# danielwillemsen/alphazero-openspiel

Hardware: AMD Instinct MI355X
Metric: self-play games/sec (higher is better)
Workload: dtype f32-grade (f16x3: split-fp16 operands, 3 MFMAs per product, fp32 accumulate); 1 GPU; connect_four, 400 sims/move, 10-block x 50-filter ResNet, 4096 concurrent games per GPU; overlap=1, weights=random-init (torch.manual_seed), eval-mode BN, net_backend=fused, tree_dtype=f64, parallelism=games sharded over 1 GPU(s), no collective inside the search, hip_graph=True, ticks_per_graph=16, workload_key=connect_four|4096|400|10|50|fused|random|f32x|1|16|build:5fb6d05c6dce

## Files before the change

### alphazero-openspiel_amd/csrc/az_head.h

```cpp
#pragma once
#include "az_head_params.h"

__device__ __forceinline__ half8 frag_from_rows(half8 v, int lane) {
    typedef int i32x4 __attribute__((ext_vector_type(4)));
    const int src = (4 * (lane & 15) + (lane >> 4)) * 4;
    i32x4 u = __builtin_bit_cast(i32x4, v);
#pragma unroll
    for (int i = 0; i < 4; i++) u[i] = __builtin_amdgcn_ds_bpermute(src, u[i]);
    return __builtin_bit_cast(half8, u);
}

template <bool X3> __global__ __launch_bounds__(HEAD_NW * 64) void az_head_kernel(HeadParams p) {
    extern __shared__ __attribute__((aligned(16))) unsigned char lds[];
    float *part = (float *)lds;
    float *logits = (float *)(lds + HEAD_NW * OTG * 64 * 16);
    const int tid = threadIdx.x, lane = tid & 63, wave = tid >> 6;
    const int b0 = blockIdx.x * 16;
    const int K = p.K, NP = p.n_ot * 16;
    int row = b0 + (lane >> 2);
    if (row >= p.n_boards) row = p.n_boards - 1;
    const _Float16 *xrow = p.x + (size_t)row * K + 8 * (lane & 3);
    const _Float16 *xrow_lo = X3 ? p.x_lo + (size_t)row * K + 8 * (lane & 3) : nullptr;
    for (int og = 0; og < p.n_ot; og += OTG) {
        f32x4 acc[OTG], acc2[X3 ? OTG : 1];
#pragma unroll
        for (int o = 0; o < OTG; o++) acc[o] = (f32x4){0.f, 0.f, 0.f, 0.f};
#pragma unroll
        for (int o = 0; o < (X3 ? OTG : 1); o++) acc2[o] = (f32x4){0.f, 0.f, 0.f, 0.f};
        if (p.n_ot == 1) {
#pragma unroll 8
            for (int ks = wave; ks < p.ksteps; ks += HEAD_NW) {
                half8 a = frag_from_rows(*(const half8 *)(xrow + 32 * ks), lane);
                half8 w = *(const half8 *)(p.fc_w + ((size_t)ks * 64 + lane) * 8);
                acc[0] = __builtin_amdgcn_mfma_f32_16x16x32_f16(a, w, acc[0], 0, 0, 0);
                if constexpr (X3) {
                    half8 al = frag_from_rows(*(const half8 *)(xrow_lo + 32 * ks), lane);
                    half8 wl = *(const half8 *)(p.fc_w_lo + ((size_t)ks * 64 + lane) * 8);
                    acc2[0] = __builtin_amdgcn_mfma_f32_16x16x32_f16(a, wl, acc2[0], 0, 0, 0);
                    acc2[0] = __builtin_amdgcn_mfma_f32_16x16x32_f16(al, w, acc2[0], 0, 0, 0);
                }
            }
        } else
        for (int ks = wave; ks < p.ksteps; ks += HEAD_NW) {
            half8 a = frag_from_rows(*(const half8 *)(xrow + 32 * ks), lane);
            half8 al;
            if constexpr (X3) al = frag_from_rows(*(const half8 *)(xrow_lo + 32 * ks), lane);
#pragma unroll
            for (int o = 0; o < OTG; o++)
                if (og + o < p.n_ot) {
                    const size_t wi = (((size_t)(og + o) * p.ksteps + ks) * 64 + lane) * 8;
                    half8 w = *(const half8 *)(p.fc_w + wi);
                    acc[o] = __builtin_amdgcn_mfma_f32_16x16x32_f16(a, w, acc[o], 0, 0, 0);
                    if constexpr (X3) {
                        half8 wl = *(const half8 *)(p.fc_w_lo + wi);
                        acc2[o] = __builtin_amdgcn_mfma_f32_16x16x32_f16(a, wl, acc2[o], 0, 0, 0);
                        acc2[o] = __builtin_amdgcn_mfma_f32_16x16x32_f16(al, w, acc2[o], 0, 0, 0);
                    }
                }
        }
#pragma unroll
        for (int o = 0; o < OTG; o++) {
            if constexpr (X3) acc[o] = acc[o] + acc2[o] * (1.0f / 2048.0f);
            *(f32x4 *)(part + ((wave * OTG + o) * 64 + lane) * 4) = acc[o];
        }
        __syncthreads();
        for (int s = tid; s < OTG * 64; s += HEAD_NW * 64) {
            int o = s >> 6, ln = s & 63;
            if (og + o >= p.n_ot) continue;
            f32x4 v = *(f32x4 *)(part + ((0 * OTG + o) * 64 + ln) * 4);
#pragma unroll
            for (int w = 1; w < HEAD_NW; w++) v += *(f32x4 *)(part + ((w * OTG + o) * 64 + ln) * 4);
            int col = 16 * (og + o) + (ln & 15);
            float bias = p.fc_b[col];
#pragma unroll
            for (int r = 0; r < 4; r++) logits[((ln >> 4) * 4 + r) * NP + col] = v[r] + bias;
        }
        __syncthreads();
    }
    const int brd = (tid >> 4) & 15, sub = tid & 15;
    const float *lg = logits + brd * NP;
    float mx = -INFINITY;
    for (int o = sub; o < p.A; o += 16) mx = fmaxf(mx, lg[o]);
#pragma unroll
    for (int off = 8; off; off >>= 1) mx = fmaxf(mx, __shfl_xor(mx, off, 16));
    float sum = 0.f;
    for (int o = sub; o < p.A; o += 16) sum += X3 ? expf(lg[o] - mx) : __expf(lg[o] - mx);
#pragma unroll
    for (int off = 8; off; off >>= 1) sum += __shfl_xor(sum, off, 16);
    if (tid < 256 && b0 + brd < p.n_boards) {
        float *out = p.priors + (size_t)(b0 + brd) * p.A;
        if (X3) {
            for (int o = sub; o < p.A; o += 16) out[o] = expf(lg[o] - mx) / sum;
        } else {
            float inv = 1.f / sum;
            for (int o = sub; o < p.A; o += 16) out[o] = __expf(lg[o] - mx) * inv;
        }
        if (sub == 0) p.values[b0 + brd] = tanhf(lg[p.A]);
    }
}

#define HG_BT 8
#define HG_OT 8
#define HG_KSPLIT 2
#define HG_RING 4
#ifndef HG_LOADERS
#define HG_LOADERS 4
#endif
template <bool X3> __global__ __launch_bounds__((8 + HG_LOADERS) * 64) void az_head_gemm_kernel(HeadParams p, float *__restrict__ logits_g) {
    extern __shared__ __attribute__((aligned(16))) unsigned char lds[];
    constexpr int NPART = X3 ? 2 : 1;
    constexpr int PIECES = (HG_BT + HG_OT) * NPART;
    constexpr int SLOT_B = PIECES * 1024;
    constexpr int NLOAD = HG_LOADERS;
    constexpr int PER = PIECES / NLOAD;
    static_assert((NLOAD == 2 || NLOAD == 4) && PIECES % NLOAD == 0 && HG_BT == 8 && HG_OT == 8 && (HG_RING - 2) * PER < 64, "piece f = NLOAD i + loader; the counted waits fit vmcnt");
    const int tid = threadIdx.x, lane = tid & 63, wave = __builtin_amdgcn_readfirstlane(tid >> 6), q = lane >> 4, l15 = lane & 15;
    const int wm = (wave & 7) >> 1, wn = (wave ^ (wave >> 2)) & 1;
    const int n_cg = (p.n_ot + HG_OT - 1) / HG_OT, ot_per = (p.n_ot + n_cg - 1) / n_cg, per_bt = n_cg * HG_KSPLIT;
    const int lin = blockIdx.x, xcd = lin & 7, j = lin >> 3;
    const int bt = (j / per_bt) * 8 + xcd;
    if (bt * 16 * HG_BT >= p.n_boards) return;
    const int og = ((j % per_bt) / HG_KSPLIT) * ot_per, kh = (j % per_bt) % HG_KSPLIT;
    const int n_og = p.n_ot - og < ot_per ? p.n_ot - og : ot_per;
    const int K = p.K, NP = p.n_ot * 16;
    const int ks_per = (p.ksteps + HG_KSPLIT - 1) / HG_KSPLIT, ks0 = kh * ks_per;
    const int nk = (p.ksteps - ks0 < ks_per ? p.ksteps - ks0 : ks_per);
    const bool loader = wave >= 8;
    const _Float16 *src0[PER];
    int kstride[PER], dst[PER];
    if (loader) {
#pragma unroll
        for (int i = 0; i < PER; i++) {
            const int f = NLOAD * i + (wave & (NLOAD - 1));
            dst[i] = f * 1024;
            if (f < HG_BT * NPART) {
                const int r = lane >> 2;
                int row = (bt * HG_BT + f % HG_BT) * 16 + r;
                if (row >= p.n_boards) row = p.n_boards - 1;
                src0[i] = (f / HG_BT ? p.x_lo : p.x) + (size_t)row * K + 8 * ((lane & 3) ^ ((r >> 3) << 1));
                kstride[i] = 32;
            } else {
                const int g = f - HG_BT * NPART;
                int ot = og + g % HG_OT;
                ot = ot < p.n_ot ? ot : p.n_ot - 1;
                src0[i] = (g / HG_OT ? p.fc_w_lo : p.fc_w) + ((size_t)ot * p.ksteps * 64 + lane) * 8;
                kstride[i] = 512;
            }
        }
    }
    auto issue = [&](int ks, int slot) {
#pragma unroll
        for (int i = 0; i < PER; i++)
            __builtin_amdgcn_global_load_lds((const __attribute__((address_space(1))) void *)(src0[i] + (size_t)ks * kstride[i]),
                                             (__attribute__((address_space(3))) void *)(lds + slot * SLOT_B + dst[i]), 16, 0, 0);
    };
    if (loader) {
#pragma unroll
        for (int s = 0; s < HG_RING - 1; s++)
            if (s < nk) issue(ks0 + s, s);
        for (int i = -1; i < nk; i++) {
            if (i + 1 < nk) {
                const int younger = nk - 2 - i < HG_RING - 2 ? nk - 2 - i : HG_RING - 2;
                static_for<HG_RING - 1>([&](auto y_c) {
                    constexpr int y = decltype(y_c)::value;
                    if (younger == y) asm volatile("s_waitcnt vmcnt(%0)" ::"n"(y * PER) : "memory");
                });
            }
            __builtin_amdgcn_s_barrier();
            asm volatile("" ::: "memory");
            if (i + HG_RING < nk) issue(ks0 + i + HG_RING, (i + HG_RING) % HG_RING);
        }
        return;
    }
    const int n_m = (bt * HG_BT + 2 * wm + 1) * 16 < p.n_boards ? 2 : (bt * HG_BT + 2 * wm) * 16 < p.n_boards ? 1 : 0;
    const int n_o = n_og - 4 * wn < 0 ? 0 : n_og - 4 * wn > 4 ? 4 : n_og - 4 * wn;
    float bias_o[4];
#pragma unroll
    for (int o = 0; o < 4; o++) bias_o[o] = kh == 0 && o < n_o ? p.fc_b[16 * (og + 4 * wn + o) + l15] : 0.f;
    f32x4 acc[2][4], acc2[X3 ? 2 : 1][X3 ? 4 : 1];
#pragma unroll
    for (int m = 0; m < 2; m++)
#pragma unroll
        for (int o = 0; o < 4; o++) {
            acc[m][o] = (f32x4){0.f, 0.f, 0.f, 0.f};
            if constexpr (X3) acc2[m][o] = (f32x4){0.f, 0.f, 0.f, 0.f};
        }
    const int a_off = (4 * l15 + (q ^ ((l15 >> 3) << 1))) * 16 + 2 * wm * 1024;
    const int w_off = (HG_BT * NPART + 4 * wn) * 1024 + lane * 16;
    auto kloop = [&](auto no_c) {
        constexpr int NO = decltype(no_c)::value, NOT = NO ? NO : 4;
        half8 af[2], afl[X3 ? 2 : 1], w[4], wl[X3 ? 4 : 1];
        auto read = [&](int i) {
            const unsigned char *sb = lds + (i % HG_RING) * SLOT_B;
#pragma unroll
            for (int m = 0; m < 2; m++) {
                af[m] = *(const half8 *)(sb + a_off + m * 1024);
                if constexpr (X3) afl[m] = *(const half8 *)(sb + a_off + (HG_BT + m) * 1024);
            }
#pragma unroll
            for (int o = 0; o < NOT; o++) {
                w[o] = *(const half8 *)(sb + w_off + o * 1024);
                if constexpr (X3) wl[o] = *(const half8 *)(sb + w_off + (HG_OT + o) * 1024);
            }
        };
        auto step = [&](int i) {
            read(i);
#pragma unroll
            for (int pass = 0; pass < (X3 ? 3 : 1); pass++)
#pragma unroll
                for (int o = 0; o < NOT; o++)
#pragma unroll
                    for (int m = 0; m < 2; m++)
// ... 76 lines not shown
```

### alphazero-openspiel_amd/csrc/az_head_params.h

```cpp
#pragma once
#include "az_net_common.h"

struct HeadParams {
    int HW, A, n_ot, ksteps, n_boards;
    int K;
    const _Float16 *x;
    const _Float16 *fc_w;
    const _Float16 *x_lo, *fc_w_lo;
    const float *fc_b;
    float *priors, *values;
};

#define OTG 8
#define HEAD_NW 8

hipError_t az_launch_tower_f16(int device, int nt, int ck, int waves, int r3, const TowerParams &tp, int grid, int lds, hipStream_t st);
hipError_t az_launch_tower_f16c(int device, int ck, const TowerParams &tp, int n_boards, int lds, hipStream_t st);
hipError_t az_launch_tower_x3(int device, int nt, bool rp1, int r3, const TowerParams &tp, int grid, int lds, hipStream_t st);
hipError_t az_launch_tower_x3b(int device, const TowerParams &tp, int grid, hipStream_t st);
hipError_t az_launch_tower_x3d(int device, int variant, const TowerParams &tp, int grid, hipStream_t st);
struct X3DVariant { int pc, tiles, rs, R; };
constexpr int AZ_X3D_VARIANTS = 3;
constexpr X3DVariant az_x3d_variant(int v) { return v == 0 ? X3DVariant{480, 18, 8, 58} : v == 1 ? X3DVariant{416, 16, 9, 84} : X3DVariant{480, 21, 8, 57}; }
hipError_t az_launch_tower_x3c(int device, int bpw, const TowerParams &tp, int n_boards, hipStream_t st);
hipError_t az_launch_head(int device, bool x3, const HeadParams &hp, int n_boards, int lds_head, float *logits, hipStream_t st);
```

### alphazero-openspiel_amd/csrc/az_net.hip

```cpp
#include <hip/hip_runtime.h>
#include <stdint.h>
#include <string.h>

#include <algorithm>
#include <cmath>

#include <string>
#include <vector>

#include "../../include/az_engine.h"
#include "../../include/az_net.h"

#include "az_net_common.h"
#include "az_head_params.h"
#include "az_net_wide.h"

#define AZ_X3C_MAX_BOARDS 512
#define AZ_F16C_MAX_BOARDS 512
#define AZ_X3C_ONE_PER_WG 256

enum class NetScheme {
    F16,
    F16C,
    X3,
// ... 284 lines not shown
    if (out.variant < 0) return out;
    const X3DVariant V = az_x3d_variant(out.variant);
    const int ncol = 16 * V.tiles;
    out.pos.assign(ncol, 0);
    std::vector<int> col_of((size_t)out.nb * HW, -1), seen(16, 0);
    for (int b = 0; b < out.nb; b++)
        for (int pp = 0; pp < HW; pp++) {
            const int r = (b * out.R + (pp / W + 1) * out.rs + pp % W + 1) & 15, k = seen[r]++;
            out.pos[k * 16 + r] = (uint16_t)(b << 8 | pp);
            col_of[(size_t)b * HW + pp] = k * 16 + r;
        }
    out.sdst.assign((size_t)ncol * 8, 0xFFFF);
    for (int col = 0; col < ncol; col++) {
        const int b = out.pos[col] >> 8, pp = out.pos[col] & 255, y = pp / W, x = pp % W;
        for (int t = 0; t < 8; t++) {
            const int tap = X3D::tap_of_plane(t), dy = tap / 3 - 1, dx = tap % 3 - 1, yd = y - dy, xd = x - dx;
            if (yd >= 0 && yd < H && xd >= 0 && xd < W) out.sdst[(size_t)col * 8 + t] = (uint16_t)col_of[(size_t)b * HW + yd * W + xd];
        }
    }
    return out;
}

static std::vector<uint16_t> repack_fc(const uint16_t *src, int n_ot, int fc_ksteps, int HW, int xc) {
    const int ks64 = HW * AZ_NET_XOUT_C / 32;
    std::vector<uint16_t> dst((size_t)n_ot * fc_ksteps * 64 * 8, 0);
    for (int ot = 0; ot < n_ot; ot++)
        for (int ks = 0; ks < fc_ksteps; ks++)
            for (int lane = 0; lane < 64; lane++)
                for (int e = 0; e < 8; e++) {
                    const int k = 32 * ks + 8 * (lane >> 4) + e;
                    if (k >= HW * xc) continue;
                    const int k64 = (k / xc) * AZ_NET_XOUT_C + k % xc;
                    dst[(((size_t)ot * fc_ksteps + ks) * 64 + lane) * 8 + e] =
                        src[(((size_t)ot * ks64 + k64 / 32) * 64 + ((k64 % 32) / 8) * 16 + (lane & 15)) * 8 + k64 % 8];
                }
    return dst;
}

template <bool IS_FIRST> static constexpr int x3b_mfma_per_tile() {
    int n = 0;
    for (int ks = 0; ks < X3BK<IS_FIRST, 1>::NKSC; ks++) n += X3BK<IS_FIRST, 1>::n_mfma(ks);
    return n;
}
static_assert(x3b_mfma_per_tile<false>() == 147, "az_tower_x3b.h: 147 against 180");
static double x3_mfma_per_wave(int nt, int n_convs, int nks) { return 3.0 * (AZ_NET_K0STEPS + (double)(n_convs - 1) * nks) * 4 * nt; }

static std::string head_label(const az_net *n) {
    const std::string t = n->precision == AZ_NET_PREC_F16X3 ? "<X3>" : "";
    return n->n_ot > OTG ? "az_head_gemm_kernel" + t + " + az_head_softmax_kernel" + t : "az_head_kernel" + t;
}
static std::string kind_label(const az_net *n, TowerKind k) {
    std::string s = TOWER_NAME[(int)k];
    if (k == TowerKind::WIDE) s += std::string(n->precision == AZ_NET_PREC_F16X3 ? "<X3>" : "<F16>") + " x" + std::to_string(2 * n->d.n_blocks);
    return k == TowerKind::X3C_FUSED_HEAD ? s : s + " + " + head_label(n);
}

template <class Desc> static int check_args(const Desc *desc, az_net **out, const char *desc_name) {
    if (!desc || !out) {
        g_net_err = "null argument";
        return AZ_E_INVALID;
    }
    *out = nullptr;
    if (desc->struct_size != (int32_t)sizeof(Desc)) {
        g_net_err = std::string(desc_name) + ".struct_size mismatch";
        return AZ_E_INVALID;
    }
    return AZ_OK;
}
static int new_net(int device, az_net **n) {
    const hipError_t s = hipSetDevice(device);
    if (s != hipSuccess) {
        g_net_err = std::string("hipSetDevice: ") + hipGetErrorString(s);
        return AZ_E_HIP;
    }
    *n = new az_net();
    return AZ_OK;
}
struct Upload {
    int rc = AZ_OK;
    void fail(int code, const char *msg) {
        if (rc != AZ_OK) return;
        g_net_err = msg;
        rc = code;
    }
    template <class T> void operator()(T *&dst, const void *src, size_t bytes) {
        if (rc == AZ_OK && (hipMalloc((void **)&dst, bytes) != hipSuccess || hipMemcpy(dst, src, bytes, hipMemcpyHostToDevice) != hipSuccess))
            fail(AZ_E_NOMEM, "hipMalloc/hipMemcpy of the net's weights failed");
    }
};
static int finish_create(az_net *n, const Upload &up, az_net **out) {
    if (up.rc != AZ_OK) {
        az_net_destroy(n);
        return up.rc;
    }
    for (int k = 0; k < N_TOWER_KINDS; k++) n->labels[k] = kind_label(n, (TowerKind)k);
    *out = n;
    return AZ_OK;
}

extern "C" int az_net_create(const az_net_desc *desc, az_net **out) {
    if (int rc = check_args(desc, out, "az_net_desc")) return rc;
    const az_net_desc &d = *desc;
    if (d.rows < 3 || d.cols < 3 || d.rows * d.cols > 64 || d.in_planes < 1 || d.in_planes > 4 || d.n_filters < 1 ||
        d.n_filters > AZ_NET_CPAD || d.n_blocks < 1 || d.num_actions < 1 || !d.conv_w || !d.conv_epi || !d.in_affine ||
        !d.skip_w || !d.fc_w || !d.fc_b) {
        g_net_err = "bad net description (need 3<=rows,cols, rows*cols<=64, in_planes<=4, n_filters<=56, packed buffers)";
        return AZ_E_INVALID;
    }
    if (d.precision != AZ_NET_PREC_F16 && d.precision != AZ_NET_PREC_F16X3) {
        g_net_err = "precision must be AZ_NET_PREC_F16 or AZ_NET_PREC_F16X3";
        return AZ_E_INVALID;
    }
    const bool x3 = d.precision == AZ_NET_PREC_F16X3;
    if (x3 && (!d.conv_w_lo || !d.fc_w_lo)) {
        g_net_err = "AZ_NET_PREC_F16X3 needs conv_w_lo and fc_w_lo";
        return AZ_E_INVALID;
    }
    const int r3 = d.n_filters <= 50 ? 2 : 16, HW = d.rows * d.cols;
    NetScheme scheme;
    X3DLayout xd;
    if (x3) {
        const TowerGeom g = x3_geom(d.rows, d.cols, r3);
        const bool x3b = g.rp1 && r3 == 2;
        if (!x3b && (g.nt > 4 || g.lds > 160 * 1024)) {
            g_net_err = "board / filter count does not fit the f16x3 tower kernel's LDS budget";
            return AZ_E_INVALID;
        }
        if (r3 == 2) xd = x3d_layout(d.rows, d.cols);
        scheme = xd.variant >= 0 ? (x3b ? NetScheme::X3B_X3D : NetScheme::X3D) : x3b ? NetScheme::X3B : NetScheme::X3;
    } else {
        const TowerGeom gc = tower_geom(1, 1, d.rows, d.cols);
        scheme = r3 == 2 && gc.tpb && gc.rs == 8 && gc.tpb <= 3 ? NetScheme::F16C : NetScheme::F16;
    }
    int best = 0;
    for (int bpw = 1; bpw <= 8; bpw++) {
        TowerGeom g = tower_geom(bpw, 4, d.rows, d.cols);
        if (g.nt > 4 || g.lds > 160 * 1024) break;
        best = bpw;
    }
    if (!best) {
        g_net_err = "board does not fit the tower kernel's LDS budget";
        return AZ_E_INVALID;
    }
    az_net *n;
    if (int rc = new_net(d.device, &n)) return rc;
    n->d = d;
    n->precision = d.precision;
    n->scheme = scheme;
    n->r3 = r3;
    memcpy(n->in_affine, d.in_affine, sizeof n->in_affine);
    n->bpw_max = best;
    n->n_ot = (d.num_actions + 1 + 15) / 16;
    n->lds_head = HEAD_NW * OTG * 64 * 16 + 16 * n->n_ot * 16 * 4;
    n->xc = (n->n_ot > OTG && HW % 2 == 0 && d.n_filters <= 52) ? 52 : AZ_NET_XOUT_C;
    n->fc_ksteps = (HW * n->xc + 31) / 32;
    Upload up;
    const int n_convs = 2 * d.n_blocks;
    auto x3_stream = [&](const X3Stream &L, _Float16 *&dst) {
        std::vector<unsigned char> s;
        if (!build_x3_stream(L, d.conv_w, d.conv_w_lo, n_convs, s))
            up.fail(AZ_E_INVALID, "AZ_NET_PREC_F16X3: a conv weight of magnitude >= 32 (the device copy holds the weights x 2048 in fp16)");
        up(dst, s.data(), s.size());
    };
    if (xd.variant >= 0) {
        n->xd_variant = xd.variant, n->xd_nb = xd.nb, n->xd_R = xd.R, n->xd_rs = xd.rs;
        x3_stream(x3d_stream_layout(), n->conv_w_d);
        up(n->xd_pos, xd.pos.data(), xd.pos.size() * 2);
        up(n->xd_sdst, xd.sdst.data(), xd.sdst.size() * 2);
    }
    if (scheme == NetScheme::X3B || scheme == NetScheme::X3B_X3D) x3_stream(x3b_stream_layout(), n->conv_w);
    else {
        const std::vector<unsigned char> s = conv_stream(d, r3);
        up(n->conv_w, s.data(), s.size());
    }
    {
        std::vector<float> e4((size_t)n_convs * 256, 0.f);
        for (int c = 0; c < n_convs; c++) {
            memcpy(&e4[(size_t)c * 256], d.conv_epi + (size_t)c * 192, 192 * sizeof(float));
            if (c + 1 < n_convs) memcpy(&e4[(size_t)c * 256 + 192], d.conv_epi + (size_t)(c + 1) * 192, 64 * sizeof(float));
            if (x3)
                for (int i = 0; i < 64; i++) e4[(size_t)c * 256 + 192 + i] *= X3_WSCALE;
        }
        up(n->epi, e4.data(), e4.size() * sizeof(float));
    }
    const size_t fw = (size_t)n->n_ot * n->fc_ksteps * 64 * 8 * 2;
    for (int lo = 0; lo < (x3 ? 2 : 1); lo++) {
        const uint16_t *src = lo ? d.fc_w_lo : d.fc_w;
        std::vector<uint16_t> re;
        if (n->xc != AZ_NET_XOUT_C) re = repack_fc(src, n->n_ot, n->fc_ksteps, HW, n->xc), src = re.data();
        up(lo ? n->fc_w_lo : n->fc_w, src, fw);
    }
    up(n->fc_b, d.fc_b, (size_t)n->n_ot * 16 * 4);
    up(n->skip_w, d.skip_w, 64 * 4 * sizeof(float));
    n->d.conv_w_lo = nullptr;
    n->d.fc_w_lo = nullptr;
    n->d.conv_w = nullptr;
    n->d.conv_epi = nullptr;
    n->d.in_affine = nullptr;
    n->d.skip_w = nullptr;
    n->d.fc_w = nullptr;
    n->d.fc_b = nullptr;
    return finish_create(n, up, out);
}

static int wide_fpad(int f) { return (f + 31) & ~31; }
static int wide_nks(const az_net *n, int conv) { return conv == 0 ? 9 : 9 * n->fpad / 32; }

extern "C" int az_net_create_wide(const az_net_wide_desc *desc, az_net **out) {
    if (int rc = check_args(desc, out, "az_net_wide_desc")) return rc;
    const az_net_wide_desc &d = *desc;
    if (d.rows < 1 || d.cols < 1 || d.rows * d.cols > 64 || d.in_planes < 1 || d.in_planes > 4 || d.n_filters < 1 ||
        d.n_filters > AZ_NET_WIDE_MAX_FILTERS || d.n_blocks < 1 || d.num_actions < 1 || d.num_actions > 768 || !d.conv_w ||
        !d.conv_b || !d.bn1_scale || !d.bn1_shift || !d.skip_w || !d.fc_w || !d.fc_b) {
        g_net_err = "bad wide net description (need rows*cols<=64, 1<=in_planes<=4, 1<=n_filters<=256, A<=768, all buffers)";
        return AZ_E_INVALID;
    }
    if (d.precision != AZ_NET_PREC_F16 && d.precision != AZ_NET_PREC_F16X3) {
        g_net_err = "precision must be AZ_NET_PREC_F16 or AZ_NET_PREC_F16X3";
        return AZ_E_INVALID;
    }
    const int F = d.n_filters, HW = d.rows * d.cols, cin0 = d.in_planes, C = F > cin0 ? F : cin0, nc = 2 * d.n_blocks;
    const int fpad = wide_fpad(F), nmt = fpad / 16, A1 = d.num_actions + 1;
    const size_t n_w = (size_t)nc * F * C * 9;
    for (size_t i = 0; i < n_w; i++)
        if (!std::isfinite(d.conv_w[i])) {
            g_net_err = "az_net_create_wide: a conv weight is not finite";
            return AZ_E_INVALID;
        }
    az_net *n;
    if (int rc = new_net(d.device, &n)) return rc;
    n->d = az_net_desc{};
    n->d.struct_size = sizeof(az_net_desc);
    n->d.rows = d.rows, n->d.cols = d.cols, n->d.in_planes = cin0, n->d.n_filters = F, n->d.n_blocks = d.n_blocks;
    n->d.num_actions = d.num_actions, n->d.device = d.device, n->d.precision = d.precision;
    n->precision = d.precision;
    n->scheme = NetScheme::WIDE;
    n->fpad = fpad;
    n->nbw = 16 * WIDE_NT / HW;
    n->xc = fpad;
    n->n_ot = (A1 + 15) / 16;
    n->fc_ksteps = HW * fpad / 32;
    n->lds_head = HEAD_NW * OTG * 64 * 16 + 16 * n->n_ot * 16 * 4;
    std::vector<uint16_t> w;
    std::vector<float> epi((size_t)nc * 4 * fpad, 0.f);
    auto h16 = [](double v) {
        _Float16 h = (_Float16)v;
        uint16_t b;
        memcpy(&b, &h, 2);
        return b;
    };
    for (int c = 0; c < nc; c++) {
        n->w_off.push_back(w.size());
        const int cin = c == 0 ? WIDE_CIN0 : fpad, n_ch = cin / 32, cin_real = c == 0 ? cin0 : F;
        const float *wc = d.conv_w + (size_t)c * F * C * 9;
        std::vector<double> sc(fpad, 1.0);
        for (int co = 0; co < F; co++) {
            double m = 0;
            for (int k = 0; k < cin_real * 9; k++) m = std::max(m, (double)std::fabs(wc[((size_t)co * C + k / 9) * 9 + k % 9]));
            int e = 0;
            if (m > 0) {
                (void)std::frexp(m, &e);
                e = std::min(100, std::max(-100, 4 - e));
            }
            sc[co] = std::ldexp(1.0, e);
        }
        const size_t base = w.size();
        w.resize(base + (size_t)n_ch * 9 * nmt * 2 * 512, 0);
        for (int ch = 0; ch < n_ch; ch++)
            for (int tap = 0; tap < 9; tap++)
                for (int mt = 0; mt < nmt; mt++)
                    for (int lane = 0; lane < 64; lane++)
                        for (int j = 0; j < 8; j++) {
                            const int co = 16 * mt + (lane & 15), ci = 32 * ch + 8 * (lane >> 4) + j;
                            if (co >= F || ci >= cin_real) continue;
                            const double v = (double)wc[((size_t)co * C + ci) * 9 + tap] * sc[co];
                            const double hi = (double)(_Float16)v;
                            const size_t o = base + ((((size_t)(ch * 9 + tap) * nmt + mt) * 2) * 512) + lane * 8 + j;
                            w[o] = h16(hi * 2048.0);
                            w[o + 512] = h16((v - hi) * 2048.0);
                        }
        float *e4 = &epi[(size_t)c * 4 * fpad];
        for (int co = 0; co < fpad; co++) e4[co] = (float)(1.0 / (2048.0 * sc[co]));
        for (int co = 0; co < F; co++) {
            e4[fpad + co] = d.conv_b[(size_t)c * F + co];
            if (c % 2 == 1 && c + 1 < nc) {
                e4[2 * fpad + co] = d.bn1_scale[(size_t)(c / 2 + 1) * C + co];
                e4[3 * fpad + co] = d.bn1_shift[(size_t)(c / 2 + 1) * C + co];
            }
        }
    }
    std::vector<float> in((size_t)8 + (size_t)fpad * 4, 0.f);
    for (int c = 0; c < cin0; c++) in[c] = d.bn1_scale[c], in[4 + c] = d.bn1_shift[c];
    for (int co = 0; co < F; co++)
        for (int c = 0; c < cin0; c++) in[8 + (size_t)co * 4 + c] = d.skip_w[(size_t)co * cin0 + c];
    const size_t fw = (size_t)n->n_ot * n->fc_ksteps * 512;
    std::vector<uint16_t> fh(fw, 0), fl(fw, 0);
    for (int ot = 0; ot < n->n_ot; ot++)
        for (int ks = 0; ks < n->fc_ksteps; ks++)
            for (int lane = 0; lane < 64; lane++)
                for (int j = 0; j < 8; j++) {
                    const int o = 16 * ot + (lane & 15), k = 32 * ks + 8 * (lane >> 4) + j, pos = k / fpad, c = k % fpad;
                    if (o >= A1 || c >= F) continue;
                    const double v = d.fc_w[(size_t)o * F * HW + (size_t)c * HW + pos], hi = (double)(_Float16)v;
                    const size_t i = (((size_t)ot * n->fc_ksteps + ks) * 64 + lane) * 8 + j;
                    fh[i] = h16(hi);
                    fl[i] = h16((v - hi) * 2048.0);
                }
    std::vector<float> fb((size_t)n->n_ot * 16, 0.f);
    for (int o = 0; o < A1; o++) fb[o] = d.fc_b[o];
    Upload up;
    up(n->w_wide, w.data(), w.size() * 2);
    up(n->epi_wide, epi.data(), epi.size() * 4);
    up(n->in_wide, in.data(), in.size() * 4);
    up(n->fc_w, fh.data(), fw * 2);
    up(n->fc_w_lo, fl.data(), fw * 2);
    up(n->fc_b, fb.data(), fb.size() * 4);
    return finish_create(n, up, out);
}

static double wide_mfma_per_board(const az_net *n, int n_boards) {
    const int HW = n->d.rows * n->d.cols, nc = 2 * n->d.n_blocks, per = n->precision == AZ_NET_PREC_F16X3 ? 3 : 1;
    double ks = 0;
    for (int c = 0; c < nc; c++) ks += wide_nks(n, c);
    const long full = n_boards / n->nbw, rest = n_boards % n->nbw;
    const double tiles = (double)full * ((n->nbw * HW + 15) / 16) + (rest ? (rest * HW + 15) / 16 : 0);
    return per * ks * (n->fpad / 16) * tiles / n_boards + per * (double)n->n_ot * n->fc_ksteps / 16.0;
}
static int wide_reserve(az_net *n, int32_t max_boards) {
    const size_t cells = (size_t)max_boards * n->d.rows * n->d.cols;
    float **fbufs[] = {&n->x_wide, &n->logits};
    for (float **b : fbufs) (void)hipFree(*b), *b = nullptr;
    _Float16 **hbufs[] = {&n->opa_hi, &n->opa_lo, &n->opb_hi, &n->opb_lo};
    for (_Float16 **b : hbufs) (void)hipFree(*b), *b = nullptr;
    n->max_boards = 0;
    NCHK(n, hipMalloc((void **)&n->x_wide, cells * n->fpad * 4));
    for (_Float16 **b : hbufs) {
        if (n->precision != AZ_NET_PREC_F16X3 && (b == &n->opa_lo || b == &n->opb_lo)) continue;
        NCHK(n, hipMalloc((void **)b, cells * n->fpad * 2));
        NCHK(n, hipMemset(*b, 0, cells * n->fpad * 2));
    }
    if (n->n_ot > OTG) NCHK(n, hipMalloc((void **)&n->logits, (size_t)max_boards * n->n_ot * 16 * sizeof(float) * 2));
    n->max_boards = max_boards;
    return AZ_OK;
}
static hipError_t wide_tower(az_net *n, const float *obs, int32_t n_boards, hipStream_t st) {
    const bool x3 = n->precision == AZ_NET_PREC_F16X3;
    const int HW = n->d.rows * n->d.cols, nc = 2 * n->d.n_blocks;
    WideInputParams ip;
    ip.HW = HW, ip.cin = n->d.in_planes, ip.fpad = n->fpad, ip.n_boards = n_boards;
    ip.obs = obs, ip.in_scale = n->in_wide, ip.in_shift = n->in_wide + 4, ip.skip_w = n->in_wide + 8;
    ip.x = n->x_wide, ip.a_hi = n->opb_hi, ip.a_lo = x3 ? n->opb_lo : nullptr;
    hipError_t s = az_launch_wide_input(ip, st);
    for (int c = 0; c < nc && s == hipSuccess; c++) {
        WideConvParams p;
        p.W = n->d.cols, p.HW = HW, p.nbw = n->nbw, p.n_boards = n_boards;
        p.cin = c == 0 ? WIDE_CIN0 : n->fpad, p.n_chunks = p.cin / 32;
        p.fpad = n->fpad, p.nmt = n->fpad / 16;
        p.mode = c % 2 == 0 ? WIDE_MODE_CONV1 : c + 1 < nc ? WIDE_MODE_CONV2 : WIDE_MODE_LAST;
        const bool in_a = c % 2 == 1;
        p.a_hi = in_a ? n->opa_hi : n->opb_hi, p.a_lo = in_a ? n->opa_lo : n->opb_lo;
        p.o_hi = in_a ? n->opb_hi : n->opa_hi, p.o_lo = in_a ? n->opb_lo : n->opa_lo;
        p.w = n->w_wide + n->w_off[c], p.epi = n->epi_wide + (size_t)c * 4 * n->fpad, p.x = n->x_wide;
        s = az_launch_wide_conv(n->d.device, x3, p, st);
    }
    return s;
}

extern "C" int az_net_reserve(az_net *n, int32_t max_boards) {
    if (!n || max_boards < 1) return AZ_E_INVALID;
    NCHK(n, hipSetDevice(n->d.device));
    if (n->scheme == NetScheme::WIDE) return wide_reserve(n, max_boards);
    if (n->xout) (void)hipFree(n->xout);
    n->xout = nullptr;
    size_t bytes = (size_t)max_boards * n->d.rows * n->d.cols * n->xc * 2 + 64;
    NCHK(n, hipMalloc((void **)&n->xout, bytes));
    NCHK(n, hipMemset(n->xout, 0, bytes));
    if (n->xout_lo) (void)hipFree(n->xout_lo);
    n->xout_lo = nullptr;
    if (n->precision == AZ_NET_PREC_F16X3) {
        NCHK(n, hipMalloc((void **)&n->xout_lo, bytes));
        NCHK(n, hipMemset(n->xout_lo, 0, bytes));
    }
    if (n->logits) (void)hipFree(n->logits);
    n->logits = nullptr;
    if (n->n_ot > OTG) NCHK(n, hipMalloc((void **)&n->logits, (size_t)max_boards * n->n_ot * 16 * sizeof(float) * 2));
    n->max_boards = max_boards;
    return AZ_OK;
}

static TowerGeom choose_geom(const az_net *n, int n_boards) {
    TowerGeom g = tower_geom(1, 4, n->d.rows, n->d.cols);
    double best_cost = -1;
    for (int bpw = 1; bpw <= n->bpw_max; bpw++)
        for (int waves = 4; waves <= 8; waves += 4) {
            TowerGeom c = tower_geom(bpw, waves, n->d.rows, n->d.cols);
            if (c.lds > 160 * 1024 || (waves == 8 && c.nt > 3)) continue;
            long wgs = (n_boards + waves * bpw - 1) / (waves * bpw);
            long rounds = (wgs + 255) / 256;
            double cost = rounds * (2.0 * (c.nt < 3 ? 3 : c.nt) + 1.0) * (waves == 8 ? 1.5 : 1.0);
            if (best_cost < 0 || cost < best_cost) {
                best_cost = cost;
                g = c;
            }
        }
    return g;
}

struct ForwardPlan {
    TowerKind kind;
    TowerGeom g = {};
    int per_wg = 0;
    int grid = 0;
    int xd_variant = -1;
    bool head = true;
};
static ForwardPlan plan_forward(const az_net *n, int n_boards) {
    ForwardPlan p;
    const int H = n->d.rows, W = n->d.cols;
    switch (n->scheme) {
    case NetScheme::WIDE:
        p.kind = TowerKind::WIDE;
        return p;
    case NetScheme::F16C:
        if (n_boards <= AZ_F16C_MAX_BOARDS) {
            p.kind = TowerKind::F16C;
            p.g = tower_geom(1, 1, H, W);
            p.g.ck = n_boards <= AZ_X3C_ONE_PER_WG ? 8 : 4;
            p.g.off_epi = (p.g.ck == 8 ? 4 : 3) * p.g.ck * 4096;
            p.g.off_act = p.g.off_epi + 2048 + 8 * 64 * 8;
            p.g.lds = p.g.off_act + N_OCT * p.g.rcells * OCT_B;
            p.per_wg = 1;
            break;
        }
        [[fallthrough]];
    case NetScheme::F16:
        p.kind = TowerKind::F16;
        p.g = choose_geom(n, n_boards);
        p.per_wg = p.g.waves * p.g.bpw;
        break;
    default: {
        const bool x3b = n->scheme == NetScheme::X3B || n->scheme == NetScheme::X3B_X3D;
        p.g = x3_geom(H, W, n->r3);
        p.per_wg = 4;
        if (x3b && n_boards <= AZ_X3C_MAX_BOARDS) {
            p.head = !(n->n_ot == 1 && n->fc_ksteps <= 96 && W >= 4);
            p.kind = p.head ? TowerKind::X3C : TowerKind::X3C_FUSED_HEAD;
            p.per_wg = n_boards > AZ_X3C_ONE_PER_WG ? 2 : 1;
        } else if (n->scheme == NetScheme::X3D || (n->scheme == NetScheme::X3B_X3D && n_boards > 128 * n->xd_nb)) {
            p.kind = TowerKind::X3D;
            p.per_wg = n->xd_nb;
            p.xd_variant = n->xd_variant;
        } else
            p.kind = x3b ? TowerKind::X3B : TowerKind::X3;
    }
    }
    p.grid = (n_boards + p.per_wg - 1) / p.per_wg;
    return p;
}

static TowerParams tower_params(const az_net *n, const ForwardPlan &p, const float *obs, float *priors, float *values, int n_boards) {
    TowerParams tp = {};
    tp.H = n->d.rows, tp.W = n->d.cols, tp.HW = tp.H * tp.W, tp.cin = n->d.in_planes, tp.n_convs = 2 * n->d.n_blocks;
    tp.n_boards = n_boards;
    tp.cells = p.g.cells, tp.rs = p.g.rs, tp.tpb = p.g.tpb, tp.bpw = p.g.bpw, tp.rcells = p.g.rcells, tp.zcell = p.g.zcell;
    tp.off_epi = p.g.off_epi, tp.off_act = p.g.off_act;
    tp.conv_w = p.kind == TowerKind::X3D ? n->conv_w_d : n->conv_w;
    tp.epi = n->epi, tp.skip_w = n->skip_w;
    memcpy(tp.in_scale, n->in_affine, 32);
    memcpy(tp.in_shift, n->in_affine + 8, 32);
    tp.obs = obs, tp.xout = n->xout, tp.xout_lo = n->xout_lo, tp.xout_c = n->xc;
    tp.fc_w = p.kind == TowerKind::X3C_FUSED_HEAD ? n->fc_w : nullptr;
    tp.fc_w_lo = n->fc_w_lo, tp.fc_b = n->fc_b, tp.priors = priors, tp.values = values;
    tp.A = n->d.num_actions, tp.fc_ksteps = n->fc_ksteps;
    tp.xd_nb = n->xd_nb, tp.xd_R = n->xd_R, tp.xd_rs = n->xd_rs, tp.xd_pos = n->xd_pos, tp.xd_sdst = n->xd_sdst;
    return tp;
}
static HeadParams head_params(const az_net *n, float *priors, float *values, int n_boards) {
    const bool wide = n->scheme == NetScheme::WIDE;
    HeadParams hp;
    hp.HW = n->d.rows * n->d.cols, hp.A = n->d.num_actions, hp.n_ot = n->n_ot, hp.K = hp.HW * n->xc, hp.ksteps = n->fc_ksteps;
    hp.n_boards = n_boards;
    hp.x = wide ? n->opb_hi : n->xout, hp.x_lo = wide ? n->opb_lo : n->xout_lo;
    hp.fc_w = n->fc_w, hp.fc_w_lo = n->fc_w_lo, hp.fc_b = n->fc_b;
    hp.priors = priors, hp.values = values;
    return hp;
}

extern "C" int az_net_issued_mfma_per_board(const az_net *n, int32_t n_boards, double *out) {
    if (!n || !out || n_boards < 1) return AZ_E_INVALID;
    const ForwardPlan p = plan_forward(n, n_boards);
    const int n_convs = 2 * n->d.n_blocks, nks = n->r3 < 16 ? 15 : AZ_NET_KSTEPS;
    const double head = (double)n->n_ot * n->fc_ksteps / 16.0;
    const double per_tile = x3b_mfma_per_tile<true>() + (double)(n_convs - 1) * x3b_mfma_per_tile<false>();
    switch (p.kind) {
    case TowerKind::F16: {
        const int nt = p.g.nt < 3 ? 3 : (p.g.nt > 3 ? 4 : 3);
        *out = (double)(AZ_NET_K0STEPS + (n_convs - 1) * nks) * 4 * nt / p.g.bpw + head;
        break;
    }
    case TowerKind::F16C:
        *out = (double)(AZ_NET_K0STEPS + (n_convs - 1) * nks) * 4 * 3 + head;
        break;
    case TowerKind::X3:
        *out = x3_mfma_per_wave(p.g.nt <= 3 ? 3 : 4, n_convs, nks) + 3.0 * head;
        break;
    case TowerKind::X3B:
    case TowerKind::X3C:
        *out = 3.0 * per_tile + 3.0 * head;
        break;
    case TowerKind::X3C_FUSED_HEAD:
        *out = 3.0 * per_tile + 3.0 * (head * 16.0 / p.per_wg);
        break;
    case TowerKind::X3D:
        *out = az_x3d_variant(p.xd_variant).tiles * per_tile / p.per_wg + 3.0 * head;
        break;
    case TowerKind::WIDE:
        *out = wide_mfma_per_board(n, n_boards);
        break;
    }
    return AZ_OK;
}

extern "C" const char *az_net_kernel_label(const az_net *n, int32_t n_boards) {
    if (!n) return "";
    return n->labels[(int)plan_forward(n, n_boards < 1 ? n->max_boards : n_boards).kind].c_str();
}

extern "C" int az_net_forward(az_net *n, const float *obs, float *priors, float *values, int32_t n_boards, void *stream) {
    if (!n || !obs || !priors || !values || n_boards < 1) return AZ_E_INVALID;
    if (n_boards > n->max_boards) {
        n->err = "n_boards exceeds az_net_reserve()";
        return AZ_E_STATE;
    }
    NCHK(n, hipSetDevice(n->d.device));
    hipStream_t st = (hipStream_t)stream;
    const ForwardPlan p = plan_forward(n, n_boards);
    const TowerParams tp = tower_params(n, p, obs, priors, values, n_boards);
    const int dv = n->d.device;
    const bool x3 = n->precision == AZ_NET_PREC_F16X3;
    hipError_t s = hipSuccess;
    switch (p.kind) {
    case TowerKind::F16: s = az_launch_tower_f16(dv, p.g.nt, p.g.ck, p.g.waves, n->r3, tp, p.grid, p.g.lds, st); break;
    case TowerKind::F16C: s = az_launch_tower_f16c(dv, p.g.ck, tp, n_boards, p.g.lds, st); break;
    case TowerKind::X3: s = az_launch_tower_x3(dv, p.g.nt, p.g.rp1, n->r3, tp, p.grid, p.g.lds, st); break;
    case TowerKind::X3B: s = az_launch_tower_x3b(dv, tp, p.grid, st); break;
    case TowerKind::X3C:
    case TowerKind::X3C_FUSED_HEAD: s = az_launch_tower_x3c(dv, p.per_wg, tp, n_boards, st); break;
    case TowerKind::X3D: s = az_launch_tower_x3d(dv, p.xd_variant, tp, p.grid, st); break;
    case TowerKind::WIDE: s = wide_tower(n, obs, n_boards, st); break;
    }
    if (s != hipSuccess) {
        n->err = std::string(p.kind == TowerKind::WIDE ? "wide tower launch: " : x3 ? "f16x3 tower launch: " : "tower launch: ") + hipGetErrorString(s);
        return AZ_E_HIP;
    }
    if (p.head) NCHK(n, az_launch_head(dv, x3, head_params(n, priors, values, n_boards), n_boards, n->lds_head, n->logits, st));
    return AZ_OK;
}

extern "C" int az_net_read_tower(az_net *n, float *out, int32_t n_boards) {
    if (!n || !out || n_boards < 1 || n_boards > n->max_boards) return AZ_E_INVALID;
    NCHK(n, hipSetDevice(n->d.device));
    NCHK(n, hipDeviceSynchronize());
    if (n->scheme == NetScheme::WIDE) {
        const size_t cnt = (size_t)n_boards * n->d.rows * n->d.cols * n->fpad;
        std::vector<_Float16> h(cnt);
        NCHK(n, hipMemcpy(h.data(), n->opb_hi, cnt * 2, hipMemcpyDeviceToHost));
        for (size_t i = 0; i < cnt; i++) out[i] = (float)h[i];
        if (n->precision == AZ_NET_PREC_F16X3) {
            NCHK(n, hipMemcpy(h.data(), n->opb_lo, cnt * 2, hipMemcpyDeviceToHost));
            for (size_t i = 0; i < cnt; i++) out[i] += (float)h[i] * (1.0f / 2048.0f);
        }
        return AZ_OK;
    }
    const size_t cells = (size_t)n_boards * n->d.rows * n->d.cols, cnt = cells * n->xc;
    const int nc = n->xc < AZ_NET_XOUT_C ? n->xc : AZ_NET_XOUT_C;
    std::vector<_Float16> h(cnt);
    NCHK(n, hipMemcpy(h.data(), n->xout, cnt * 2, hipMemcpyDeviceToHost));
    for (size_t i = 0; i < cells * AZ_NET_XOUT_C; i++) out[i] = 0.f;
    for (size_t c = 0; c < cells; c++)
        for (int ch = 0; ch < nc; ch++) out[c * AZ_NET_XOUT_C + ch] = (float)h[c * n->xc + ch];
    if (n->precision == AZ_NET_PREC_F16X3) {
        NCHK(n, hipMemcpy(h.data(), n->xout_lo, cnt * 2, hipMemcpyDeviceToHost));
        for (size_t c = 0; c < cells; c++)
            for (int ch = 0; ch < nc; ch++) out[c * AZ_NET_XOUT_C + ch] += (float)h[c * n->xc + ch] * (1.0f / 2048.0f);
    }
    return AZ_OK;
}
```

### alphazero-openspiel_amd/csrc/az_net_common.h

```cpp
#pragma once
#include <hip/hip_runtime.h>
#include <stdint.h>

#include <type_traits>
#include <utility>

#include "../../include/az_net.h"

typedef _Float16 half8 __attribute__((ext_vector_type(8)));
typedef _Float16 half4 __attribute__((ext_vector_type(4)));
typedef float f32x4 __attribute__((ext_vector_type(4)));

#define OCT_B 16
#define AZ_NET_K0STEPS 4
#define N_OCT 7
#define AZ_MAX_DEVICES 64
#define X3_LOFF_RP1 (N_OCT * 96 * OCT_B)

struct TowerParams {
    int H, W, HW, cells, cin, n_convs, n_boards, bpw;
    int rcells;
    int zcell;
    int rs;
    int tpb;
    int off_epi;
    int off_act;
    const _Float16 *conv_w;
    const float *epi;
    const float *skip_w;
    float in_scale[8], in_shift[8];
    const float *obs;
    _Float16 *xout;
    _Float16 *xout_lo;
    int xout_c;
    const _Float16 *fc_w, *fc_w_lo;
    const float *fc_b;
    float *priors, *values;
    int A, fc_ksteps;
    int xd_nb, xd_R, xd_rs;
    const uint16_t *xd_pos;
    const uint16_t *xd_sdst;
};

__device__ __forceinline__ float lrelu(float v) { return fmaxf(v, 0.01f * v); }

__device__ __forceinline__ half4 lrelu_h4(half4 h) { return __builtin_elementwise_max(h, h * (_Float16)0.01f); }
__device__ __forceinline__ int opaque(int v) {
    asm volatile("" : "+v"(v));
    return v;
}
__device__ __forceinline__ void wait_lgkm(int n) {
    switch (n < 15 ? n : 15) {
    case 0: asm volatile("s_waitcnt lgkmcnt(0)" ::: "memory"); break;
    case 1: asm volatile("s_waitcnt lgkmcnt(1)" ::: "memory"); break;
    case 2: asm volatile("s_waitcnt lgkmcnt(2)" ::: "memory"); break;
    case 3: asm volatile("s_waitcnt lgkmcnt(3)" ::: "memory"); break;
    case 4: asm volatile("s_waitcnt lgkmcnt(4)" ::: "memory"); break;
    case 5: asm volatile("s_waitcnt lgkmcnt(5)" ::: "memory"); break;
    case 6: asm volatile("s_waitcnt lgkmcnt(6)" ::: "memory"); break;
    case 7: asm volatile("s_waitcnt lgkmcnt(7)" ::: "memory"); break;
    case 8: asm volatile("s_waitcnt lgkmcnt(8)" ::: "memory"); break;
    case 9: asm volatile("s_waitcnt lgkmcnt(9)" ::: "memory"); break;
    case 10: asm volatile("s_waitcnt lgkmcnt(10)" ::: "memory"); break;
    case 11: asm volatile("s_waitcnt lgkmcnt(11)" ::: "memory"); break;
    case 12: asm volatile("s_waitcnt lgkmcnt(12)" ::: "memory"); break;
    case 13: asm volatile("s_waitcnt lgkmcnt(13)" ::: "memory"); break;
    case 14: asm volatile("s_waitcnt lgkmcnt(14)" ::: "memory"); break;
    default: asm volatile("s_waitcnt lgkmcnt(15)" ::: "memory"); break;
    }
}
__device__ __forceinline__ void lds_read128(half8 &dst, unsigned lds_byte_addr) {
    asm volatile("ds_read_b128 %0, %1" : "=v"(dst) : "v"(lds_byte_addr));
}
template <int OFF> __device__ __forceinline__ void lds_read128_off(half8 &dst, unsigned lds_byte_addr) {
    static_assert(OFF >= 0 && OFF < 65536, "ds offset field is 16 bits");
    asm volatile("ds_read_b128 %0, %1 offset:%2" : "=v"(dst) : "v"(lds_byte_addr), "n"(OFF));
}
template <int OFF> __device__ __forceinline__ void lds_read_f4_off(f32x4 &dst, unsigned lds_byte_addr) {
    asm volatile("ds_read_b128 %0, %1 offset:%2" : "=v"(dst) : "v"(lds_byte_addr), "n"(OFF));
}
__device__ __forceinline__ void keep_alive(const f32x4 &v) { asm volatile("" ::"v"(v)); }
__device__ __forceinline__ void launder(half8 &v) { asm volatile("" : "+v"(v)); }
__device__ __forceinline__ void launder(f32x4 &v) { asm volatile("" : "+v"(v)); }
typedef float f32x2 __attribute__((ext_vector_type(2)));
__device__ __forceinline__ void launder(f32x2 &v) { asm volatile("" : "+v"(v)); }
__device__ __forceinline__ void launder_u(unsigned &v) { asm volatile("" : "+v"(v)); }
__device__ __forceinline__ void pin_acc(f32x4 &v) { asm volatile("" : "+a"(v)); }
__device__ __forceinline__ void split_pair(float x0, float x1, unsigned &hi, unsigned &lo) {
    const float m = -2048.0f, t0 = x0 * 2048.0f, t1 = x1 * 2048.0f;
    asm("v_cvt_pk_f16_f32 %0, %1, %2" : "=v"(hi) : "v"(x0), "v"(x1));
    asm("v_fma_mixlo_f16 %0, %1, %2, %3 op_sel_hi:[1,0,0]" : "=&v"(lo) : "v"(hi), "v"(m), "v"(t0));
    asm("v_fma_mixhi_f16 %0, %1, %2, %3 op_sel:[1,0,0] op_sel_hi:[1,0,0]" : "+v"(lo) : "v"(hi), "v"(m), "v"(t1));
}
__device__ __forceinline__ void split_pair_planes(float x0, float x1, unsigned &hi, unsigned &lo0) {
    const float m = -1.0f;
    asm("v_cvt_pk_f16_f32 %0, %1, %2" : "=v"(hi) : "v"(x0), "v"(x1));
    asm("v_fma_mixlo_f16 %0, %1, %2, %3 op_sel_hi:[1,0,0]" : "=&v"(lo0) : "v"(hi), "v"(m), "v"(x0));
    asm("v_fma_mixhi_f16 %0, %1, %2, %3 op_sel:[1,0,0] op_sel_hi:[1,0,0]" : "+v"(lo0) : "v"(hi), "v"(m), "v"(x1));
}
__device__ __forceinline__ void split4_planes(const f32x4 &v, half4 &hi, half4 &lo0) {
    typedef unsigned u32x2 __attribute__((ext_vector_type(2)));
    unsigned h0, h1, l0, l1;
    split_pair_planes(v[0], v[1], h0, l0);
    split_pair_planes(v[2], v[3], h1, l1);
    hi = __builtin_bit_cast(half4, (u32x2){h0, h1});
    lo0 = __builtin_bit_cast(half4, (u32x2){l0, l1});
}
#define X3_WSCALE 2048.0f
__device__ __forceinline__ void split4_f16x3(const f32x4 &v, half4 &hi, half4 &lo) {
    typedef unsigned u32x2 __attribute__((ext_vector_type(2)));
    unsigned h0, h1, l0, l1;
    split_pair(v[0], v[1], h0, l0);
    split_pair(v[2], v[3], h1, l1);
    hi = __builtin_bit_cast(half4, (u32x2){h0, h1});
    lo = __builtin_bit_cast(half4, (u32x2){l0, l1});
}
__device__ __forceinline__ f32x4 comb_f16x3(const f32x4 &a, const f32x4 &a2) {
    const f32x4 is = {1.0f / 2048.0f, 1.0f / 2048.0f, 1.0f / 2048.0f, 1.0f / 2048.0f};
    return __builtin_elementwise_fma(a2, is, a);
}
__device__ __forceinline__ unsigned addr_add(unsigned a, unsigned b) {
    unsigned r;
    asm volatile("v_add_u32 %0, %1, %2" : "=v"(r) : "v"(a), "v"(b));
    return r;
}
template <int OFF> __device__ __forceinline__ void lds_read64_off(f32x2 &dst, unsigned lds_byte_addr) {
    asm volatile("ds_read_b64 %0, %1 offset:%2" : "=v"(dst) : "v"(lds_byte_addr), "n"(OFF));
}
__device__ __forceinline__ void lds_write64(unsigned lds_byte_addr, f32x2 v) { asm volatile("ds_write_b64 %0, %1" ::"v"(lds_byte_addr), "v"(v) : "memory"); }
template <int OFF> __device__ __forceinline__ void lds_write64_off(unsigned lds_byte_addr, f32x2 v) {
    asm volatile("ds_write_b64 %0, %1 offset:%2" ::"v"(lds_byte_addr), "v"(v), "n"(OFF) : "memory");
}
#define READ_A(dst, addr, off) lds_read128_off<(off)>(dst, addr)
template <int OFF> __device__ __forceinline__ void lds_read32_off(unsigned &dst, unsigned lds_byte_addr) {
    asm volatile("ds_read_b32 %0, %1 offset:%2" : "=v"(dst) : "v"(lds_byte_addr), "n"(OFF));
}
#define READ_B32_OFF(dst, addr, off) lds_read32_off<(off)>(dst, addr)
#define READ_B(dst, addr) lds_read128(dst, addr)
#define READ_B_OFF(dst, addr, off) lds_read128_off<(off)>(dst, addr)
constexpr int x3b_part_bytes(int part) { return part == 1 ? 4 * 6144 + 6 * 1024 : part == 3 ? 3 * 6144 + 1024 : 4 * 6144; }
constexpr int x3b_part_off(int part) { return part == 0 ? 0 : x3b_part_off(part - 1) + x3b_part_bytes(part - 1); }
struct X3B {
    static constexpr int FR = 1024;
    static constexpr int REC2 = 6 * FR;
    static constexpr int CK = 4, NKS = 15, PARTS = 4;
    static constexpr int part_bytes(int part) { return x3b_part_bytes(part); }
    static constexpr int part_off(int part) { return x3b_part_off(part); }
    static constexpr int CONV_B = x3b_part_off(3) + x3b_part_bytes(3);
    static constexpr int C0_B = AZ_NET_K0STEPS * REC2 + AZ_NET_K0STEPS * FR;
    static constexpr int CHUNK_S = x3b_part_bytes(1);
    static constexpr int S_PLANE = 48 * 8, S_WAVE = 9 * S_PLANE;
    static constexpr int PLANE_B = 96 * OCT_B;
    static constexpr int LO_OFF = 6 * PLANE_B + 96 * 4;
    static constexpr int OFF_EPI = 2 * CHUNK_S;
    static constexpr int OFF_S = OFF_EPI + 2048 + 256 * 16;
    static constexpr int OFF_ACT = OFF_S + 4 * S_WAVE;
    static constexpr int LDS = OFF_ACT + 4 * 2 * LO_OFF;
    static constexpr int tap_of_plane(int t) { return t < 4 ? t : t + 1; }
    template <int PART> static constexpr int n_pieces() { return (PART < 0 ? C0_B : x3b_part_bytes(PART < 0 ? 0 : PART)) / 1024; }
    template <int PART> static constexpr size_t chunk_off(int c) {
        return PART < 0 ? 0 : (size_t)C0_B + (size_t)((c - 1) / PARTS) * CONV_B + x3b_part_off(PART < 0 ? 0 : PART);
    }
    static constexpr int extra_off(bool is_first, int ks) {
        return is_first ? AZ_NET_K0STEPS * REC2 + ks * FR : (ks / CK == 1 ? 4 * REC2 + (ks - 6) * 3 * FR : 3 * REC2);
    }
};
template <bool IS_FIRST, int NT> struct X3BK {
    static constexpr int NKSC = IS_FIRST ? AZ_NET_K0STEPS : X3B::NKS;
// ... 99 lines not shown
```

Baseline: 1437 games/s.

## Store trunk output at 52-channel stride and read it in the head with masked tail

The trunk output buffer now uses a 52-channel stride whenever the board size is even and the filter count fits, not only for large action heads. For small heads such as connect_four, the head kernel keeps the original 64-channel-padded FC weight layout and reads the activations at 26-half strides, with odd waves masking off the tail octets. The aim is to shrink the activation buffer the tower writes and the head reads. The cost is more complex addressing, unaligned 8-byte vector loads, and an extra per-wave mode branch.

New measurement: 1440 games/s (median of 6 runs). About the same (+0.3%).

```diff
diff --git a/alphazero-openspiel_amd/csrc/az_head.h b/alphazero-openspiel_amd/csrc/az_head.h
--- a/alphazero-openspiel_amd/csrc/az_head.h
+++ b/alphazero-openspiel_amd/csrc/az_head.h
@@ -10,54 +10,78 @@
     return __builtin_bit_cast(half8, u);
 }
 
+typedef half8 half8_a8 __attribute__((aligned(8)));
+__device__ __forceinline__ half8 trunk52_tail(half8 v, int octet) {
+    typedef unsigned u32x4 __attribute__((ext_vector_type(4)));
+    const u32x4 u = __builtin_bit_cast(u32x4, v);
+    const unsigned keep = octet < 2 ? ~0u : 0u, down = octet == 2 ? ~0u : 0u;
+    return __builtin_bit_cast(half8, (u32x4){(u[0] & keep) | (u[2] & down), (u[1] & keep) | (u[3] & down), u[2] & keep, u[3] & keep});
+}
+
 template <bool X3> __global__ __launch_bounds__(HEAD_NW * 64) void az_head_kernel(HeadParams p) {
     extern __shared__ __attribute__((aligned(16))) unsigned char lds[];
+    static_assert(HEAD_NW % 2 == 0, "a wave keeps one half of every position (trunk52_tail)");
     float *part = (float *)lds;
     float *logits = (float *)(lds + HEAD_NW * OTG * 64 * 16);
-    const int tid = threadIdx.x, lane = tid & 63, wave = tid >> 6;
+    const int tid = threadIdx.x, lane = tid & 63, wave = __builtin_amdgcn_readfirstlane(tid >> 6);
     const int b0 = blockIdx.x * 16;
     const int K = p.K, NP = p.n_ot * 16;
     int row = b0 + (lane >> 2);
     if (row >= p.n_boards) row = p.n_boards - 1;
-    const _Float16 *xrow = p.x + (size_t)row * K + 8 * (lane & 3);
-    const _Float16 *xrow_lo = X3 ? p.x_lo + (size_t)row * K + 8 * (lane & 3) : nullptr;
+    const bool c52 = p.xc == AZ_NET_TRUNK_C, tail = c52 && (wave & 1);
+    const int octet = lane & 3;
+    const int lane_off = c52 ? (32 - AZ_NET_TRUNK_C / 2) * (wave & 1) + (tail && octet >= 2 ? 12 : 8 * octet) : 8 * octet;
+    const _Float16 *xrow = p.x + (size_t)row * K + lane_off;
+    const _Float16 *xrow_lo = X3 ? p.x_lo + (size_t)row * K + lane_off : nullptr;
     for (int og = 0; og < p.n_ot; og += OTG) {
         f32x4 acc[OTG], acc2[X3 ? OTG : 1];
 #pragma unroll
         for (int o = 0; o < OTG; o++) acc[o] = (f32x4){0.f, 0.f, 0.f, 0.f};
 #pragma unroll
         for (int o = 0; o < (X3 ? OTG : 1); o++) acc2[o] = (f32x4){0.f, 0.f, 0.f, 0.f};
-        if (p.n_ot == 1) {
+        auto kloop = [&](auto mode_c) {
+            constexpr bool TAIL = decltype(mode_c)::value == 2;
+            constexpr int kstride = decltype(mode_c)::value ? AZ_NET_TRUNK_C / 2 : 32;
+            auto a_frag = [&](const _Float16 *xr, int ks) {
+                half8 v = *(const half8_a8 *)(xr + kstride * ks);
+                if constexpr (TAIL) v = trunk52_tail(v, octet);
+                return frag_from_rows(v, lane);
+            };
+            if (p.n_ot == 1) {
 #pragma unroll 8
-            for (int ks = wave; ks < p.ksteps; ks += HEAD_NW) {
-                half8 a = frag_from_rows(*(const half8 *)(xrow + 32 * ks), lane);
-                half8 w = *(const half8 *)(p.fc_w + ((size_t)ks * 64 + lane) * 8);
-                acc[0] = __builtin_amdgcn_mfma_f32_16x16x32_f16(a, w, acc[0], 0, 0, 0);
-                if constexpr (X3) {
-                    half8 al = frag_from_rows(*(const half8 *)(xrow_lo + 32 * ks), lane);
-                    half8 wl = *(const half8 *)(p.fc_w_lo + ((size_t)ks * 64 + lane) * 8);
-                    acc2[0] = __builtin_amdgcn_mfma_f32_16x16x32_f16(a, wl, acc2[0], 0, 0, 0);
-                    acc2[0] = __builtin_amdgcn_mfma_f32_16x16x32_f16(al, w, acc2[0], 0, 0, 0);
-                }
-            }
-        } else
-        for (int ks = wave; ks < p.ksteps; ks += HEAD_NW) {
-            half8 a = frag_from_rows(*(const half8 *)(xrow + 32 * ks), lane);
-            half8 al;
-            if constexpr (X3) al = frag_from_rows(*(const half8 *)(xrow_lo + 32 * ks), lane);
-#pragma unroll
-            for (int o = 0; o < OTG; o++)
-                if (og + o < p.n_ot) {
-                    const size_t wi = (((size_t)(og + o) * p.ksteps + ks) * 64 + lane) * 8;
-                    half8 w = *(const half8 *)(p.fc_w + wi);
-                    acc[o] = __builtin_amdgcn_mfma_f32_16x16x32_f16(a, w, acc[o], 0, 0, 0);
+                for (int ks = wave; ks < p.ksteps; ks += HEAD_NW) {
+                    half8 a = a_frag(xrow, ks);
+                    half8 w = *(const half8 *)(p.fc_w + ((size_t)ks * 64 + lane) * 8);
+                    acc[0] = __builtin_amdgcn_mfma_f32_16x16x32_f16(a, w, acc[0], 0, 0, 0);
                     if constexpr (X3) {
-                        half8 wl = *(const half8 *)(p.fc_w_lo + wi);
-                        acc2[o] = __builtin_amdgcn_mfma_f32_16x16x32_f16(a, wl, acc2[o], 0, 0, 0);
-                        acc2[o] = __builtin_amdgcn_mfma_f32_16x16x32_f16(al, w, acc2[o], 0, 0, 0);
+                        half8 al = a_frag(xrow_lo, ks);
+                        half8 wl = *(const half8 *)(p.fc_w_lo + ((size_t)ks * 64 + lane) * 8);
+                        acc2[0] = __builtin_amdgcn_mfma_f32_16x16x32_f16(a, wl, acc2[0], 0, 0, 0);
+                        acc2[0] = __builtin_amdgcn_mfma_f32_16x16x32_f16(al, w, acc2[0], 0, 0, 0);
                     }
                 }
-        }
+            } else
+            for (int ks = wave; ks < p.ksteps; ks += HEAD_NW) {
+                half8 a = a_frag(xrow, ks);
+                half8 al;
+                if constexpr (X3) al = a_frag(xrow_lo, ks);
+#pragma unroll
+                for (int o = 0; o < OTG; o++)
+                    if (og + o < p.n_ot) {
+                        const size_t wi = (((size_t)(og + o) * p.ksteps + ks) * 64 + lane) * 8;
+                        half8 w = *(const half8 *)(p.fc_w + wi);
+                        acc[o] = __builtin_amdgcn_mfma_f32_16x16x32_f16(a, w, acc[o], 0, 0, 0);
+                        if constexpr (X3) {
+                            half8 wl = *(const half8 *)(p.fc_w_lo + wi);
+                            acc2[o] = __builtin_amdgcn_mfma_f32_16x16x32_f16(a, wl, acc2[o], 0, 0, 0);
+                            acc2[o] = __builtin_amdgcn_mfma_f32_16x16x32_f16(al, w, acc2[o], 0, 0, 0);
+                        }
+                    }
+            }
+        };
+        if (tail) kloop(std::integral_constant<int, 2>{});
+        else if (c52) kloop(std::integral_constant<int, 1>{});
+        else kloop(std::integral_constant<int, 0>{});
 #pragma unroll
         for (int o = 0; o < OTG; o++) {
             if constexpr (X3) acc[o] = acc[o] + acc2[o] * (1.0f / 2048.0f);
diff --git a/alphazero-openspiel_amd/csrc/az_head_params.h b/alphazero-openspiel_amd/csrc/az_head_params.h
--- a/alphazero-openspiel_amd/csrc/az_head_params.h
+++ b/alphazero-openspiel_amd/csrc/az_head_params.h
@@ -4,6 +4,7 @@
 struct HeadParams {
     int HW, A, n_ot, ksteps, n_boards;
     int K;
+    int xc;
     const _Float16 *x;
     const _Float16 *fc_w;
     const _Float16 *x_lo, *fc_w_lo;
diff --git a/alphazero-openspiel_amd/csrc/az_net.hip b/alphazero-openspiel_amd/csrc/az_net.hip
--- a/alphazero-openspiel_amd/csrc/az_net.hip
+++ b/alphazero-openspiel_amd/csrc/az_net.hip
@@ -460,8 +460,9 @@
     n->bpw_max = best;
     n->n_ot = (d.num_actions + 1 + 15) / 16;
     n->lds_head = HEAD_NW * OTG * 64 * 16 + 16 * n->n_ot * 16 * 4;
-    n->xc = (n->n_ot > OTG && HW % 2 == 0 && d.n_filters <= 52) ? 52 : AZ_NET_XOUT_C;
-    n->fc_ksteps = (HW * n->xc + 31) / 32;
+    n->xc = (HW % 2 == 0 && d.n_filters <= AZ_NET_TRUNK_C) ? AZ_NET_TRUNK_C : AZ_NET_XOUT_C;
+    const bool fc_at_stride = n->n_ot > OTG && n->xc != AZ_NET_XOUT_C;
+    n->fc_ksteps = fc_at_stride ? (HW * n->xc + 31) / 32 : HW * AZ_NET_XOUT_C / 32;
     Upload up;
     const int n_convs = 2 * d.n_blocks;
     auto x3_stream = [&](const X3Stream &L, _Float16 *&dst) {
@@ -495,7 +496,7 @@
     for (int lo = 0; lo < (x3 ? 2 : 1); lo++) {
         const uint16_t *src = lo ? d.fc_w_lo : d.fc_w;
         std::vector<uint16_t> re;
-        if (n->xc != AZ_NET_XOUT_C) re = repack_fc(src, n->n_ot, n->fc_ksteps, HW, n->xc), src = re.data();
+        if (fc_at_stride) re = repack_fc(src, n->n_ot, n->fc_ksteps, HW, n->xc), src = re.data();
         up(lo ? n->fc_w_lo : n->fc_w, src, fw);
     }
     up(n->fc_b, d.fc_b, (size_t)n->n_ot * 16 * 4);
@@ -786,7 +787,7 @@
 static HeadParams head_params(const az_net *n, float *priors, float *values, int n_boards) {
     const bool wide = n->scheme == NetScheme::WIDE;
     HeadParams hp;
-    hp.HW = n->d.rows * n->d.cols, hp.A = n->d.num_actions, hp.n_ot = n->n_ot, hp.K = hp.HW * n->xc, hp.ksteps = n->fc_ksteps;
+    hp.HW = n->d.rows * n->d.cols, hp.A = n->d.num_actions, hp.n_ot = n->n_ot, hp.K = hp.HW * n->xc, hp.xc = n->xc, hp.ksteps = n->fc_ksteps;
     hp.n_boards = n_boards;
     hp.x = wide ? n->opb_hi : n->xout, hp.x_lo = wide ? n->opb_lo : n->xout_lo;
     hp.fc_w = n->fc_w, hp.fc_w_lo = n->fc_w_lo, hp.fc_b = n->fc_b;
diff --git a/alphazero-openspiel_amd/csrc/az_net_common.h b/alphazero-openspiel_amd/csrc/az_net_common.h
--- a/alphazero-openspiel_amd/csrc/az_net_common.h
+++ b/alphazero-openspiel_amd/csrc/az_net_common.h
@@ -14,6 +14,7 @@
 #define OCT_B 16
 #define AZ_NET_K0STEPS 4
 #define N_OCT 7
+#define AZ_NET_TRUNK_C 52
 #define AZ_MAX_DEVICES 64
 #define X3_LOFF_RP1 (N_OCT * 96 * OCT_B)
 
```
